# xx-peach/animatable_nerf

Measured on AMD Instinct MI355X. Metric: ray-samples/sec (512×512 rays × 64 samples) + PSNR, aninerf_s9p at 1/2/4/8 GPUs, higher is better.
Workload: dtype fp32; 1 GPU; aninerf_s9p full 512x512 render (config 2: fp32, novel-view eval, perturb=0); render_precision=fp32, rays_per_gpu=262142, samples_per_ray=64, chunk=2048, alpha_ind_rows=5863584, parallelism=replicas1 (one frame per GPU)

## Files before the change

animatable_nerf_amd/csrc/anr_mlp_body.h:

```cpp
#pragma once
#include <type_traits>

#include "anr_common.h"
#include "anr_kernels.h"
#include "anr_layers.h"

namespace anr {


template <int B, int E, typename F>
__device__ __forceinline__ void static_for(F&& f) {
  if constexpr (B < E) {
    f(std::integral_constant<int, B>{});
    static_for<B + 1, E>(f);
  }
}

typedef __attribute__((address_space(3))) void lds_void;
typedef __bf16 bf16x8 __attribute__((ext_vector_type(8)));
#ifndef ANR_FRAG_PF
#define ANR_FRAG_PF 3
#endif
#ifndef ANR_DMA_SPREAD
#define ANR_DMA_SPREAD 1
#endif
#ifndef ANR_X6_PF
#define ANR_X6_PF 2
#endif
#ifndef ANR_FAST_MATH
#define ANR_FAST_MATH 1
#endif

template <int V>
__host__ __device__ constexpr int prog_base() { return V >= 10 ? V - 10 : V; }
template <int V>
__host__ __device__ constexpr int prog_len() {
  constexpr int B = prog_base<V>();
  return B == 0 ? 30 : (B == 2 || B == 4) ? 28 : (B == 3 || B == 5) ? 9 : B == 7 ? 8 : B == 6 ? 5 : 18;
}
template <int V>
__host__ __device__ constexpr bool prog_seq() {
  return prog_base<V>() == 3 || prog_base<V>() == 5 || prog_base<V>() == 6 || prog_base<V>() == 7;
}
template <int V>
__host__ __device__ constexpr int prog_layer(int e) {
  if (V >= 10) return prog_layer<prog_base<V>()>(e);
  return V == 3 ? ANR_L_RESD0 + e
         : V == 5 ? ANR_L_SDF0 + e
         : V == 7 ? ANR_L_SREV0 + e
         : V == 6 ? ANR_L_COL0 + e
         : e < 9 ? e
         : V == 0 ? e - 9
         : (V == 2 || V == 4) ? (e < 26 ? e - 9 : (e == 26 ? ANR_L_HEAD : ANR_L_RGB))
         : V == 8 ? (e < 17 ? e : ANR_L_ALPHA)
                  : (e < 17 ? e : ANR_L_ALPHA);
}
__host__ __device__ constexpr bool prog_pose(int e) { return e < 9; }
template <bool B16, int V>
__host__ __device__ constexpr int prog_mode(int e) {
  return B16 ? ((V == 4 || V == 8 || V >= 10) ? 2 : e < 9 ? ANR_POSE_MODE : 1) : 0;
}
template <int V>
__host__ __device__ constexpr int prog_nobg(int e) { return (layer_desc_all(prog_layer<V>(e)).ob + 7) / 8; }
template <bool B16, int V>
__host__ __device__ constexpr int prog_slices(int e) {
  return prog_mode<B16, V>(e) == 2   ? ks32(prog_layer<V>(e)) * prog_nobg<V>(e)
         : prog_mode<B16, V>(e) == 1 ? ks32(prog_layer<V>(e)) + (b16_tail_ob(prog_layer<V>(e)) > 0 ? 1 : 0)
                                  : layer_ksteps(prog_layer<V>(e)) / ANR_KSLICE;
}
template <int V>
__host__ __device__ constexpr int x6_group_obs(int e, int gidx) {
  return layer_desc_all(prog_layer<V>(e)).ob - 8 * gidx < 8 ? layer_desc_all(prog_layer<V>(e)).ob - 8 * gidx : 8;
}
template <int V>
__host__ __device__ constexpr int x6_slice_of(int e, int G) {
  return (G / layer_desc_all(prog_layer<V>(e)).ob) * prog_nobg<V>(e) + (G % layer_desc_all(prog_layer<V>(e)).ob) / 8;
}
template <int V>
__host__ __device__ constexpr int x6_certified_at(int e, int F) {
  const int o = F % layer_desc_all(prog_layer<V>(e)).ob;
  const int gob = x6_group_obs<V>(e, o / 8);
  return x6_slice_of<V>(e, F) + (o % 8 > (gob - 1) / 2 ? 1 : 0);
}
template <int V>
__host__ __device__ constexpr int x6_issue_at(int e, int G) {
  int F = G - ANR_X6_PF > 0 ? G - ANR_X6_PF : 0;
  while (x6_certified_at<V>(e, F) < x6_slice_of<V>(e, G)) ++F;
  return F;
}
template <int V>
__host__ __device__ constexpr bool x6_schedule_ok(int e) {
  const int n = ks32(prog_layer<V>(e)) * layer_desc_all(prog_layer<V>(e)).ob;
  for (int G = 0; G < n; ++G) {
    const int F = x6_issue_at<V>(e, G);
    if (F > G || F < G - ANR_X6_PF) return false;
    if (x6_slice_of<V>(e, G) > x6_certified_at<V>(e, F)) return false;
    if (x6_slice_of<V>(e, G) > x6_slice_of<V>(e, F) + 1 || x6_slice_of<V>(e, G) < x6_slice_of<V>(e, F)) return false;
  }
  return true;
}
template <bool B16, int V>
__host__ __device__ constexpr int prog_slice_kb(int e, int q) {
  return prog_mode<B16, V>(e) == 2 ? x6_group_obs<V>(e, q % prog_nobg<V>(e)) * 3
         : prog_mode<B16, V>(e) == 1
             ? (q < ks32(prog_layer<V>(e)) ? b16_main_ob(prog_layer<V>(e)) * 2
                                          : b16_tail_ob(prog_layer<V>(e)) * ks32(prog_layer<V>(e)) * 2)
             : layer_chunks(prog_layer<V>(e)) * ANR_KSLICE;
}
template <bool B16, int V>
__host__ __device__ constexpr int prog_slice_off(int e, int q) {
  return prog_mode<B16, V>(e) == 2
             ? (prog_seq<V>() ? x6seq_layer_offset(prog_layer<V>(0), prog_layer<V>(e))
                              : x6_base() + x6_layer_offset(prog_layer<V>(e))) +
                   ((q / prog_nobg<V>(e)) * layer_desc_all(prog_layer<V>(e)).ob + 8 * (q % prog_nobg<V>(e))) * 3072
         : prog_mode<B16, V>(e) == 1
             ? (prog_seq<V>() ? seq_layer_offset(prog_layer<V>(0), prog_layer<V>(e))
                              : b16_base() + b16_layer_offset(prog_layer<V>(e))) +
                   q * b16_main_ob(prog_layer<V>(e)) * 2048
             : layer_offset(prog_layer<V>(e)) + q * layer_chunks(prog_layer<V>(e)) * ANR_KSLICE * 1024;
}
template <bool B16, int V>
__host__ __device__ constexpr int prog_slice_loads(int e, int q) { return (prog_slice_kb<B16, V>(e, q) + 7) / 8; }
template <bool B16, int V>
__host__ __device__ constexpr int prog_advance(int e, int q, int d) {
  for (int i = 0; i < d; ++i) {
    if (q + 1 < prog_slices<B16, V>(e)) {
      ++q;
    } else {
      q = 0;
      e = (e + 1) % prog_len<V>();
    }
  }
  return e * 1024 + q;
}
template <bool B16, int V>
__host__ __device__ constexpr int prog_later_loads(int e, int q) {
  int n = 0;
  for (int d = 1; d <= mlp_nbuf<B16>() - 3; ++d) {
    const int eq = prog_advance<B16, V>(e, q, d);
    n += prog_slice_loads<B16, V>(eq / 1024, eq % 1024);
  }
  return n;
}

template <int N>
__device__ __forceinline__ void wait_vmcnt() {
  static_assert(N >= 0 && N < 64, "vmcnt out of range");
  __builtin_amdgcn_s_waitcnt((N & 15) | (7 << 4) | (15 << 8) | ((N >> 4) << 14));
}

struct Pipe {
  unsigned char* lds;
  int smax;
  int nbuf;
  const unsigned char* wimg;
  int cur;
  int wave;
  int lane;
  int pose_woff;
  int pend;

  __device__ __forceinline__ void stage(int off, int kb, int loads, int buf, int first = 0) {
    const unsigned dst = (unsigned)(uintptr_t)(lds + buf * smax);
    const unsigned char* w = wimg;
    asm volatile("" : "+s"(w));
    for (int i = first; i < loads; ++i) {
      int piece = wave + 8 * i;
      piece = piece < kb ? piece : kb - 1;
      const unsigned m0 = dst + piece * 1024;
      const unsigned char* sbase = w + off + piece * 1024;
      asm volatile("s_mov_b32 m0, %2\n\ts_nop 0\n\tglobal_load_lds_dwordx4 %0, %1" ::"v"(lane * 16), "s"(sbase), "s"(m0)
                   : "memory");
    }
  }

  template <int N>
  __device__ __forceinline__ void wait_stream() {
    wait_vmcnt<N>();
  }

  template <bool B16, int V, int E, int Q>
  __device__ __forceinline__ void stage_slice(int buf) {
    constexpr int off = prog_slice_off<B16, V>(E, Q);
    stage(off + (prog_pose(E) ? pose_woff : 0), prog_slice_kb<B16, V>(E, Q), prog_slice_loads<B16, V>(E, Q), buf);
  }

  template <bool B16, int V>
  __device__ __forceinline__ void start() {
    static_for<0, mlp_nbuf<B16>() - 1>([&](auto d) {
      constexpr int eq = prog_advance<B16, V>(0, 0, decltype(d)::value);
      stage_slice<B16, V, eq / 1024, eq % 1024>(decltype(d)::value);
    });
    cur = 0;
    wait_stream<prog_later_loads<B16, V>(0, 0)>();
    __syncthreads();
  }

  template <bool B16, int V, int E, int Q>
  __device__ __forceinline__ const unsigned char* enter() {
    return lds + cur * smax;
  }
  template <bool B16, int V, int E, int Q, bool SPREAD = false>
  __device__ __forceinline__ void mid() {
    constexpr int NB = mlp_nbuf<B16>();
    constexpr int e1 = prog_advance<B16, V>(E, Q, 1);
    constexpr int eq = prog_advance<B16, V>(E, Q, NB - 1);
    wait_stream<prog_later_loads<B16, V>(e1 / 1024, e1 % 1024)>();
    __syncthreads();
    int slot = cur + NB - 1;
    slot = slot >= NB ? slot - NB : slot;
    if constexpr (SPREAD) pend = slot;
    else stage_slice<B16, V, eq / 1024, eq % 1024>(slot);
  }
  template <bool B16, int V, int E, int Q, int I0, int I1>
  __device__ __forceinline__ void piece() {
    constexpr int NB = mlp_nbuf<B16>();
    constexpr int eq = prog_advance<B16, V>(E, Q, NB - 1);
    constexpr int EE = eq / 1024, QQ = eq % 1024;
    constexpr int off = prog_slice_off<B16, V>(EE, QQ);
    constexpr int loads = prog_slice_loads<B16, V>(EE, QQ);
    constexpr int i1 = I1 < loads ? I1 : loads;
    if constexpr (I0 < i1) stage(off + (prog_pose(EE) ? pose_woff : 0), prog_slice_kb<B16, V>(EE, QQ), i1, pend, I0);
  }
  __device__ __forceinline__ void leave() { cur = cur + 1 >= nbuf ? 0 : cur + 1; }
};

__device__ __forceinline__ void split8(const float (&x)[8], bf16x8& hi, bf16x8& lo) {
#pragma unroll
  for (int j = 0; j < 8; ++j) {
    const __bf16 h = (__bf16)x[j];
    hi[j] = h;
    lo[j] = (__bf16)(x[j] - (float)h);
  }
}

__device__ __forceinline__ void split8x3(const float (&x)[8], bf16x8& hi, bf16x8& mid, bf16x8& lo) {
#pragma unroll
  for (int j = 0; j < 8; ++j) {
    const __bf16 h = (__bf16)x[j];
    const float r1 = x[j] - (float)h;
    const __bf16 m = (__bf16)r1;
    hi[j] = h;
    mid[j] = m;
    lo[j] = (__bf16)(r1 - (float)m);
  }
}

template <int V>
__host__ __device__ constexpr int prog_bias_off(int e) {
  int o = 0;
  for (int k = 0; k < e; ++k) o += layer_desc_all(prog_layer<V>(k)).ob * 16;
  return o;
}
static_assert(prog_bias_off<0>(prog_len<0>()) == ANR_BIAS_TABLE_FLOATS, "bias table size (anr_layers.h)");
static_assert(prog_bias_off<1>(prog_len<1>()) <= ANR_BIAS_TABLE_FLOATS, "bias table size (anr_layers.h)");
static_assert(prog_bias_off<2>(prog_len<2>()) <= ANR_BIAS_TABLE_FLOATS, "bias table size (anr_layers.h)");
static_assert(prog_bias_off<4>(prog_len<4>()) <= ANR_BIAS_TABLE_FLOATS, "bias table size (anr_layers.h)");
static_assert(prog_bias_off<8>(prog_len<8>()) <= ANR_BIAS_TABLE_FLOATS, "bias table size (anr_layers.h)");
static_assert(prog_bias_off<3>(prog_len<3>()) == seq_bias_off(ANR_L_RESD0, ANR_RESD_LAYERS), "resd bias section");
static_assert(prog_bias_off<5>(prog_len<5>()) == seq_bias_off(ANR_L_SDF0, ANR_SDF_LAYERS), "sdf bias section");
static_assert(prog_bias_off<5>(prog_len<5>()) <= ANR_BIAS_TABLE_FLOATS, "bias table size (anr_layers.h)");
static_assert(prog_bias_off<7>(prog_len<7>()) == seq_bias_off(ANR_L_SREV0, ANR_SREV_LAYERS), "sdf grad bias section");
static_assert(prog_bias_off<6>(prog_len<6>()) == seq_bias_off(ANR_L_COL0, ANR_COL_LAYERS), "colour bias section");
static_assert(prog_bias_off<7>(prog_len<7>()) + 256 <= ANR_BIAS_TABLE_FLOATS, "bias table + W8 row (anr_layers.h)");

template <int V>
__device__ __forceinline__ void fill_bias_table(const MlpArgs& a, float* __restrict__ sb, int tid) {
  static_for<0, prog_len<V>()>([&](auto ee) {
    constexpr int e = decltype(ee)::value;
    constexpr int L = prog_layer<V>(e);
    constexpr int n = layer_desc_all(L).ob * 16;
    constexpr int boff = bias_offset(L);
    constexpr int toff = prog_bias_off<V>(e);
    const float* src;
    constexpr int VB = prog_base<V>();
    if constexpr (VB == 3) {
      src = e == 0 ? a.fold : e == 5 ? a.fold + 256 : a.bias + toff;
    } else if constexpr (VB == 5 || VB == 7) {
      src = a.bias + toff;
    } else if constexpr (VB == 6) {
      src = e == 3 ? a.fold + 512 : a.bias + toff;
    } else if constexpr (e < 9) {
      src = L == 0 ? a.fold + 0 : L == 5 ? a.fold + 512 : a.bias + a.pose_boff + boff;
    } else if constexpr (V != 1 && V != 8 && e < 18) {
      src = L == 0 ? a.fold + 256 : L == 5 ? a.fold + 768 : a.bias + boff;
    } else {
      src = L == 18 ? a.fold + 1024 : L == ANR_L_HEAD ? a.fold + ANR_FOLD_HEAD : a.bias + boff;
    }
    for (int i = tid; i < n; i += 512) sb[toff + i] = src[i];
  });
}

#ifndef ANR_X3_STREAM
#define ANR_X3_STREAM 1
#endif
template <int L>
__host__ __device__ constexpr bool x3_stream_layer() {
  return ANR_X3_STREAM && b16_tail_ob(L) == 0;
}

template <int MOB, int PF>
__host__ __device__ constexpr int x3_issue_at(int G) {
  const int t = G / MOB;
  const int a = G - PF;
  if (t == 0) return a;
  const int m = (t - 1) * MOB + (MOB - 1) / 2;
  return a > m ? a : m;
}

struct LayerIO {
  float* spst = nullptr;
  const float* fst = nullptr;
  float fscale = 1.0f;
  const float* g0 = nullptr;
  const float* g1 = nullptr;
};

#ifndef ANR_SDF_NT
#define ANR_SDF_NT 1
#endif

__device__ __forceinline__ float softplus100(float x) {
  const float e = __builtin_amdgcn_exp2f(x * 144.269504f);
  const float h = __builtin_amdgcn_logf(1.0f + e) * 0.00693147181f;
  return x * 100.f > 20.f ? x : h;
}

__device__ __forceinline__ float softplus100_fac(float x, float& fac) {
  constexpr float C_HI = 144.26950073242188f, C_LO = 3.356474508109386e-06f;
  constexpr float LN2 = 0.6931471824645996f;
  const float xc = fminf(x, 0.4f);
  const float a = xc * C_HI;
  const float a_lo = __builtin_fmaf(xc, C_LO, __builtin_fmaf(xc, C_HI, -a));
  const float E = __builtin_amdgcn_exp2f(a);
  const float e = __builtin_fmaf(E, a_lo * LN2, E);
  const float u = 1.f + e;
  const float err = e - (u - 1.f);
  const float ru = __builtin_amdgcn_rcpf(u);
  fac = e * ru;
  return fmaxf(__builtin_fmaf(__builtin_amdgcn_logf(u), LN2, err * ru) * 0.01f, x);
}
template <int V>
__device__ __forceinline__ float sp_fwd(float x) {
  static_assert(V < 10, "the fp32-level programs use softplus100_fac");
  return softplus100(x);
}

template <bool B16, int V, int E, bool RELU_IN, int SP_IN, int FAC_IN, int NIN, int NOUT>
__device__ __forceinline__ void layer_x3(Pipe& p, const f32x4 (&in)[NIN], const float (&emb)[16], const float (&vemb)[8],
                                         f32x4 (&out)[NOUT], const float* __restrict__ sbias, int g, int lane,
                                         const LayerIO& io) {
  float* __restrict__ spst = io.spst;
  const float* __restrict__ fst = io.fst;
  const float fscale = io.fscale;
  constexpr int L = prog_layer<V>(E);
  constexpr LayerDesc D = layer_desc_all(L);
  constexpr int KS = ks32(L);
  constexpr int K0 = D.seg[0].ksteps / 8;
  constexpr int MOB = b16_main_ob(L);
  constexpr int PF = ANR_FRAG_PF;
  constexpr int NF = PF + 1;
  constexpr int MID = (MOB - 1) / 2;
  constexpr int BOFF = prog_bias_off<V>(E);
  static_assert(b16_tail_ob(L) == 0, "streamed x3 layers have no tail slice");
  f32x4 hv[2][2];
  auto load_h = [&](auto tc) {
    constexpr int t = decltype(tc)::value;
    if constexpr (FAC_IN != 0 && t < KS) {
#if ANR_SDF_NT
      hv[t & 1][0] = __builtin_nontemporal_load((const f32x4*)(fst + 32 * t + 4 * g));
      hv[t & 1][1] = __builtin_nontemporal_load((const f32x4*)(fst + 32 * t + 16 + 4 * g));
#else
      hv[t & 1][0] = *(const f32x4*)(fst + 32 * t + 4 * g);
      hv[t & 1][1] = *(const f32x4*)(fst + 32 * t + 16 + 4 * g);
#endif
    }
  };
// ... 224 lines not shown
          }
          load_h(std::integral_constant<int, tt + 1>{});
        }
        if constexpr (SP_IN != 0) {
          float* d = io.spst ? io.spst + 32 * ts + 4 * g : nullptr;
          const int c = 32 * ts + 4 * g;
#pragma unroll
          for (int q = 0; q < 2; ++q) {
            float f[4];
#pragma unroll
            for (int j = 0; j < 4; ++j) x[4 * q + j] = softplus100_fac(x[4 * q + j], f[j]);
            if (d) {
              if constexpr (SP_IN == 1) {
                __builtin_nontemporal_store(f32x4{f[0], f[1], f[2], f[3]}, (f32x4*)(d + 16 * q));
              } else {
#pragma unroll
                for (int j = 0; j < 4; ++j)
                  if (c + 16 * q + j < 217) d[16 * q + j] = f[j];
              }
            }
          }
        }
      }
      bf16x8 bh, bm, bl;
      split8x3(x, bh, bm, bl);
      static_for<0, OB>([&](auto ob) {
        constexpr int o = decltype(ob)::value;
        constexpr int F = tt * OB + o;
        constexpr int SQ = tt * NOBG + o / 8;
        if constexpr (o % 8 == 0) buf = p.template enter<B16, V, E, SQ>();
        if constexpr (tt == 0 && o == 0) init_bias();
        static_for<0, NS>([&](auto dd) {
          constexpr int G = F + decltype(dd)::value;
          if constexpr (G < KS * OB && x6_issue_at<V>(E, G) == F) {
            constexpr int og = G % OB;
            const unsigned char* src =
                x6_slice_of<V>(E, G) == SQ ? buf : p.lds + (p.cur + 1 >= p.nbuf ? 0 : p.cur + 1) * p.smax;
            fr[G % NS][0] = *(const bf16x8*)(src + (og % 8) * 3072 + lane * 16);
            fr[G % NS][1] = *(const bf16x8*)(src + (og % 8) * 3072 + 1024 + lane * 16);
            fr[G % NS][2] = *(const bf16x8*)(src + (og % 8) * 3072 + 2048 + lane * 16);
          }
        });
        __builtin_amdgcn_sched_barrier(0);
        const bf16x8 ah = fr[F % NS][0], am = fr[F % NS][1], al = fr[F % NS][2];
        out[o] = __builtin_amdgcn_mfma_f32_16x16x32_bf16(ah, bl, out[o], 0, 0, 0);
        out[o] = __builtin_amdgcn_mfma_f32_16x16x32_bf16(al, bh, out[o], 0, 0, 0);
        out[o] = __builtin_amdgcn_mfma_f32_16x16x32_bf16(am, bm, out[o], 0, 0, 0);
        out[o] = __builtin_amdgcn_mfma_f32_16x16x32_bf16(ah, bm, out[o], 0, 0, 0);
        out[o] = __builtin_amdgcn_mfma_f32_16x16x32_bf16(am, bh, out[o], 0, 0, 0);
        out[o] = __builtin_amdgcn_mfma_f32_16x16x32_bf16(ah, bh, out[o], 0, 0, 0);
        __builtin_amdgcn_sched_barrier(0);
        constexpr int GOB = x6_group_obs<V>(E, o / 8);
        if constexpr (o % 8 == (GOB - 1) / 2) p.template mid<B16, V, E, SQ>();
        if constexpr (o % 8 == GOB - 1) p.leave();
      });
    });
  } else if constexpr (prog_mode<B16, V>(E) != 0) {
    constexpr int KS = ks32(L);
    constexpr int K0 = D.seg[0].ksteps / 8;
    static_for<0, KS>([&](auto t) {
      constexpr int tt = decltype(t)::value;
      const unsigned char* buf = p.template enter<B16, V, E, tt>();
      if constexpr (tt == 0) init_bias();
      constexpr int seg = tt < K0 ? 0 : 1;
      constexpr int ts = tt < K0 ? tt : tt - K0;
      constexpr int kind = D.seg[seg].kind;
      float x[8];
      if constexpr (kind == SRC_EMB || kind == SRC_EMB6) {
#pragma unroll
        for (int j = 0; j < 8; ++j) x[j] = emb[8 * ts + j];
      } else if constexpr (kind == SRC_VEMB) {
#pragma unroll
        for (int j = 0; j < 8; ++j) x[j] = vemb[j];
      } else {
#pragma unroll
        for (int j = 0; j < 4; ++j) {
          x[j] = in[2 * ts][j];
          x[4 + j] = in[2 * ts + 1][j];
        }
      }
      {
        bf16x8 bh, bl;
        split8(x, bh, bl);
        constexpr int MOB = b16_main_ob(L);
        constexpr int PF = ANR_FRAG_PF;
        bf16x8 fh[PF + 1], fl[PF + 1];
        static_for<0, PF>([&](auto pp) {
          constexpr int o = decltype(pp)::value;
          if constexpr (o < MOB) {
            fh[o] = *(const bf16x8*)(buf + o * 2048 + lane * 16);
            fl[o] = *(const bf16x8*)(buf + o * 2048 + 1024 + lane * 16);
          }
        });
        static_for<0, MOB>([&](auto ob) {
          constexpr int o = decltype(ob)::value;
          constexpr int r = o % (PF + 1), rn = (o + PF) % (PF + 1);
          if constexpr (o + PF < MOB) {
            fh[rn] = *(const bf16x8*)(buf + (o + PF) * 2048 + lane * 16);
            fl[rn] = *(const bf16x8*)(buf + (o + PF) * 2048 + 1024 + lane * 16);
          }
          __builtin_amdgcn_sched_barrier(0);
          out[o] = __builtin_amdgcn_mfma_f32_16x16x32_bf16(fl[r], bh, out[o], 0, 0, 0);
          out[o] = __builtin_amdgcn_mfma_f32_16x16x32_bf16(fh[r], bl, out[o], 0, 0, 0);
          out[o] = __builtin_amdgcn_mfma_f32_16x16x32_bf16(fh[r], bh, out[o], 0, 0, 0);
          __builtin_amdgcn_sched_barrier(0);
          constexpr int MID = (MOB - 1) / 2;
          if constexpr (!ANR_DMA_SPREAD) {
            if constexpr (o == MID) p.template mid<B16, V, E, tt>();
          } else {
            constexpr int eqr = prog_advance<B16, V>(E, tt, mlp_nbuf<B16>() - 1);
            constexpr int NL = prog_slice_loads<B16, V>(eqr / 1024, eqr % 1024);
            constexpr int SPAN = MOB - 1 - MID;
            if constexpr (o == MID) p.template mid<B16, V, E, tt, true>();
            if constexpr (SPAN == 0) {
              if constexpr (o == MID) p.template piece<B16, V, E, tt, 0, NL>();
            } else if constexpr (o > MID) {
              constexpr int lo = ((o - MID - 1) * NL + SPAN - 1) / SPAN;
              constexpr int hi = o == MOB - 1 ? NL : ((o - MID) * NL + SPAN - 1) / SPAN;
              p.template piece<B16, V, E, tt, lo, hi>();
            }
          }
        });
        p.leave();
      }
    });
    if constexpr (b16_tail_ob(L) > 0) {
      constexpr int TOB = b16_tail_ob(L);
      const unsigned char* buf = p.template enter<B16, V, E, KS>();
      static_for<0, KS>([&](auto t) {
        constexpr int tt = decltype(t)::value;
        static_assert(D.nseg == 1 && D.seg[0].kind == SRC_ACT, "tail blocks only on activation-input layers");
        float x[8];
#pragma unroll
        for (int j = 0; j < 4; ++j) {
          x[j] = in[2 * tt][j];
          x[4 + j] = in[2 * tt + 1][j];
        }
        bf16x8 bh, bl;
        split8(x, bh, bl);
        static_for<0, TOB>([&](auto ob) {
          constexpr int o = decltype(ob)::value;
          const unsigned char* f = buf + (tt * TOB + o) * 2048 + lane * 16;
          const bf16x8 ah = *(const bf16x8*)f;
          const bf16x8 al = *(const bf16x8*)(f + 1024);
          out[16 + o] = __builtin_amdgcn_mfma_f32_16x16x32_bf16(al, bh, out[16 + o], 0, 0, 0);
          out[16 + o] = __builtin_amdgcn_mfma_f32_16x16x32_bf16(ah, bl, out[16 + o], 0, 0, 0);
          out[16 + o] = __builtin_amdgcn_mfma_f32_16x16x32_bf16(ah, bh, out[16 + o], 0, 0, 0);
        });
        if constexpr (tt == (KS - 1) / 2) p.template mid<B16, V, E, KS>();
      });
      p.leave();
    }
  } else {
    constexpr int C = layer_chunks(L);
    constexpr int K = layer_ksteps(L);
    constexpr int K0 = D.seg[0].ksteps;
    const unsigned char* buf = nullptr;
    static_for<0, K>([&](auto t) {
      constexpr int tt = decltype(t)::value;
      if constexpr (tt % ANR_KSLICE == 0) buf = p.template enter<B16, V, E, tt / ANR_KSLICE>();
      if constexpr (tt == 0) init_bias();
      f32x4 w[C];
      static_for<0, C>([&](auto c) {
        constexpr int cc = decltype(c)::value;
        w[cc] = *(const f32x4*)(buf + (((tt % ANR_KSLICE) * C + cc) * 64 + lane) * 16);
      });
      constexpr int seg = tt < K0 ? 0 : 1;
      constexpr int ts = tt < K0 ? tt : tt - K0;
      constexpr int kind = D.seg[seg].kind;
      float b;
      if constexpr (kind == SRC_EMB) b = emb[ts];
      else if constexpr (kind == SRC_VEMB) b = vemb[ts];
      else b = in[ts >> 2][ts & 3];
      static_for<0, D.ob>([&](auto ob) {
        constexpr int o = decltype(ob)::value;
        out[o] = __builtin_amdgcn_mfma_f32_16x16x4f32(w[o >> 2][o & 3], b, out[o], 0, 0, 0);
      });
      if constexpr (tt % ANR_KSLICE == ANR_KSLICE / 2 - 1) p.template mid<B16, V, E, tt / ANR_KSLICE>();
      if constexpr (tt % ANR_KSLICE == ANR_KSLICE - 1) p.leave();
    });
  }
  if constexpr (RELU) {
    static_for<0, D.ob>([&](auto ob) {
      constexpr int o = decltype(ob)::value;
#pragma unroll
      for (int r = 0; r < 4; ++r) out[o][r] = fmaxf(out[o][r], 0.0f);
    });
  }
}

__device__ __forceinline__ void sincos_fast(float x, float& s, float& c) {
  const float k = __builtin_rintf(x * 0.636619772367581343f);
  float r = __builtin_fmaf(-k, 1.57079601287841796875f, x);
  r = __builtin_fmaf(-k, 3.1391647326017846e-07f, r);
  r = __builtin_fmaf(-k, 5.3903025299577648e-15f, r);
  const float z = r * r;
  float ps = __builtin_fmaf(z, -1.9515295891e-4f, 8.3321608736e-3f);
  ps = __builtin_fmaf(ps, z, -1.6666654611e-1f);
  const float sn = __builtin_fmaf(ps * z, r, r);
  float pc = __builtin_fmaf(z, 2.443315711809948e-5f, -1.388731625493765e-3f);
  pc = __builtin_fmaf(pc, z, 4.166664568298827e-2f);
  pc = __builtin_fmaf(pc, z, -0.5f);
  const float cs = __builtin_fmaf(pc, z, 1.0f);
  const int q = (int)k;
  const float s0 = (q & 1) ? cs : sn, c0 = (q & 1) ? sn : cs;
  s = (q & 2) ? -s0 : s0;
  c = ((q + 1) & 2) ? -c0 : c0;
}

template <int NS>
__device__ __forceinline__ void embed_b(const float x[3], int h, int nfreq, float (&e)[8 * NS]) {
  asm volatile("" : "+v"(h));
  const float m = fmaxf(fabsf(x[0]), fmaxf(fabsf(x[1]), fabsf(x[2])));
  const bool slow = __builtin_amdgcn_ballot_w64(!(m * (float)(1 << (nfreq - 1)) <= 65536.0f)) != 0;
  const int hb = 4 * NS * h - 2;
#pragma unroll
  for (int s = 0; s < NS; ++s)
#pragma unroll
    for (int p = 0; p < 4; ++p) {
      const int P = hb + 4 * s + p;
      const int freq = (P * 11) >> 5;
      const int comp = P - 3 * freq;
      const float xc = comp == 0 ? x[0] : (comp == 1 ? x[1] : x[2]);
      const float arg = __builtin_ldexpf(xc, freq);
      float sv, cv;
      if (!slow) sincos_fast(arg, sv, cv);
      else sincosf(arg, &sv, &cv);
      const bool valid = (unsigned)P < (unsigned)(3 * nfreq);
      float v0 = valid ? sv : 0.0f, v1 = valid ? cv : 0.0f;
      if (s == 0 && p < 2) {
        const bool raw = h == 0;
        v0 = raw ? x[2 * p] : v0;
        v1 = raw ? (p == 0 ? x[1] : 0.0f) : v1;
      }
      e[8 * s + 2 * p] = v0;
      e[8 * s + 2 * p + 1] = v1;
    }
}

template <int NS>
__device__ __forceinline__ void embed(const float x[3], int g, int nfreq, float (&e)[NS]) {
#pragma unroll
  for (int s = 0; s < NS; ++s) {
    const int f = 4 * s + g;
    float v;
    if (f < 3) {
      v = x[f == 0 ? 0 : (f == 1 ? 1 : 2)];
    } else {
      const int q = f - 3;
      const int freq = q / 6;
      const int w = q - freq * 6;
      const int comp = w >= 3 ? w - 3 : w;
      const float xc = comp == 0 ? x[0] : (comp == 1 ? x[1] : x[2]);
      const float arg = xc * (float)(1 << (freq < 15 ? freq : 0));
      float sv, cv;
      sincosf(arg, &sv, &cv);
      v = freq >= nfreq ? 0.0f : (w >= 3 ? cv : sv);
    }
    e[s] = v;
  }
}

template <bool FAST = false>
__device__ __forceinline__ void lookup24(const float* __restrict__ vol32, const float p[3], const float* __restrict__ bounds,
                                         int X, int Y, int Z, int g, f32x4 (&out)[2]) {
#pragma clang fp contract(off)
  asm volatile("" : "+s"(X), "+s"(Y), "+s"(Z), "+s"(bounds));
  float lo[3], hi[3];
#pragma unroll
  for (int c = 0; c < 3; ++c) { lo[c] = bounds[c]; hi[c] = bounds[3 + c]; }
  TriCell t;
  if constexpr (FAST) {
    float gq[3];
#pragma unroll
    for (int c = 0; c < 3; ++c) gq[c] = (p[c] - lo[c]) * __builtin_amdgcn_rcpf(hi[c] - lo[c]) * 2.0f - 1.0f;
    const float ix = grid_src(gq[2], Z), iy = grid_src(gq[1], Y), iz = grid_src(gq[0], X);
    tri_cell_src(ix, iy, iz, X, Y, Z, t);
  } else {
    tri_cell(p, lo, hi, X, Y, Z, t);
  }
  f32x4 a0 = {0.f, 0.f, 0.f, 0.f}, a1 = {0.f, 0.f, 0.f, 0.f};
#pragma unroll
  for (int k = 0; k < 8; ++k) {
    if (t.base[k] >= 0) {
      const f32x4 v0 = *(const f32x4*)(vol32 + (size_t)t.base[k] * 32 + 4 * g);
      const f32x4 v1 = *(const f32x4*)(vol32 + (size_t)t.base[k] * 32 + 16 + 4 * g);
#pragma unroll
      for (int r = 0; r < 4; ++r) {
        a0[r] = a0[r] + v0[r] * t.w[k];
        a1[r] = a1[r] + v1[r] * t.w[k];
      }
    }
  }
  out[0] = a0;
  out[1] = a1;
}

template <bool FAST = false>
__device__ __forceinline__ void blend_softmax(const f32x4 (&fc)[2], const f32x4 (&init)[2], int g, f32x4 (&bw)[2]) {
  float lg[2][4];
  float m = -INFINITY;
#pragma unroll
  for (int b = 0; b < 2; ++b)
#pragma unroll
    for (int r = 0; r < 4; ++r) {
      const bool valid = b == 0 || g < 2;
      const float v = (FAST ? __logf(init[b][r] + 1e-9f) : logf(init[b][r] + 1e-9f)) + fc[b][r];
      lg[b][r] = valid ? v : -INFINITY;
      m = fmaxf(m, lg[b][r]);
    }
  m = fmaxf(m, __shfl_xor(m, 16));
  m = fmaxf(m, __shfl_xor(m, 32));
  float s = 0.f;
#pragma unroll
  for (int b = 0; b < 2; ++b)
#pragma unroll
    for (int r = 0; r < 4; ++r) {
      lg[b][r] = FAST ? __expf(lg[b][r] - m) : expf(lg[b][r] - m);
      s += lg[b][r];
    }
  s += __shfl_xor(s, 16);
  s += __shfl_xor(s, 32);
#pragma unroll
  for (int b = 0; b < 2; ++b)
#pragma unroll
    for (int r = 0; r < 4; ++r) bw[b][r] = FAST ? lg[b][r] * __builtin_amdgcn_rcpf(s) : lg[b][r] / s;
}

__device__ __forceinline__ void lbs_inverse(const f32x4 (&bw)[2], const float* __restrict__ sA, int g, const float x[3],
                                            float xt[3]) {
  float Ab[16];
#pragma unroll
  for (int m = 0; m < 16; ++m) Ab[m] = 0.f;
#pragma unroll
  for (int b = 0; b < 2; ++b)
#pragma unroll
    for (int r = 0; r < 4; ++r) {
      const int j = b * 16 + 4 * g + r;
      if (j < 24) {
        const float wj = bw[b][r];
#pragma unroll
        for (int m = 0; m < 16; ++m) Ab[m] += wj * sA[j * 16 + m];
      }
    }
#pragma unroll
  for (int m = 0; m < 16; ++m) {
    Ab[m] += __shfl_xor(Ab[m], 16);
    Ab[m] += __shfl_xor(Ab[m], 32);
  }
  const float a = Ab[0], b = Ab[1], c = Ab[2], d = Ab[4], e = Ab[5], f = Ab[6], gg = Ab[8], h = Ab[9], i = Ab[10];
  const float c00 = e * i - f * h, c01 = c * h - b * i, c02 = b * f - c * e;
  const float c10 = f * gg - d * i, c11 = a * i - c * gg, c12 = c * d - a * f;
  const float c20 = d * h - e * gg, c21 = b * gg - a * h, c22 = a * e - b * d;
  const float det = a * c00 + b * c10 + c * c20;
  const float rd = 1.0f / det;
  const float y0 = x[0] - Ab[3], y1 = x[1] - Ab[7], y2 = x[2] - Ab[11];
  xt[0] = (c00 * rd) * y0 + (c01 * rd) * y1 + (c02 * rd) * y2;
  xt[1] = (c10 * rd) * y0 + (c11 * rd) * y1 + (c12 * rd) * y2;
  xt[2] = (c20 * rd) * y0 + (c21 * rd) * y1 + (c22 * rd) * y2;
}

__device__ __forceinline__ void store_rows(float* __restrict__ rows, int idx, const f32x4 (&bw)[2], int g, bool valid) {
  if (!valid) return;
  *(f32x4*)(rows + (size_t)idx * 24 + 4 * g) = bw[0];
  if (g < 2) *(f32x4*)(rows + (size_t)idx * 24 + 16 + 4 * g) = bw[1];
}

template <bool B16, int V, int E0>
__device__ __forceinline__ void bw_mlp(Pipe& p, const float (&emb)[16], const float (&vemb)[8], const float* __restrict__ sb,
                                       f32x4 (&A)[17], f32x4 (&B)[17], f32x4 (&fc)[2], int g, int lane) {
  f32x4 dummy[1];
  layer<B16, V, E0 + 0, true>(p, dummy, emb, vemb, A, sb, g, lane);
  layer<B16, V, E0 + 1, true, true>(p, A, emb, vemb, B, sb, g, lane);
  layer<B16, V, E0 + 2, true, true>(p, B, emb, vemb, A, sb, g, lane);
  layer<B16, V, E0 + 3, true, true>(p, A, emb, vemb, B, sb, g, lane);
  layer<B16, V, E0 + 4, true, true>(p, B, emb, vemb, A, sb, g, lane);
  layer<B16, V, E0 + 5, true, true>(p, A, emb, vemb, B, sb, g, lane);
  layer<B16, V, E0 + 6, true, true>(p, B, emb, vemb, A, sb, g, lane);
  layer<B16, V, E0 + 7, true, true>(p, A, emb, vemb, B, sb, g, lane);
  layer<B16, V, E0 + 8, false, true>(p, B, emb, vemb, fc, sb, g, lane);
}

template <bool B16, int V = 2>
__device__ __forceinline__ void mlp_body(const MlpArgs& a) {
  static_assert(V == 2 || V == 4, "render programs");
  constexpr bool FAST = B16 && ANR_FAST_MATH && V == 2;
  extern __shared__ __attribute__((aligned(16))) unsigned char smem[];
  const int tid = threadIdx.x;
  const int lane = tid & 63;
  const int wave = __builtin_amdgcn_readfirstlane(tid >> 6);
  const int g = lane >> 4;
  const int pl = lane & 15;
  float* sb = (float*)smem;
  float* sA = (float*)(smem + mlp_sa_off());
  for (int i = tid; i < 384; i += 512) sA[i] = a.A[i];
  fill_bias_table<V>(a, sb, tid);

  float* sT = sA + 384;
  if (tid < 6) sT[tid] = a.tbounds[tid];
  const int n = *a.n_kept;
  const int ntiles = (n + 127) / 128;
  if ((int)blockIdx.x >= ntiles) return;

  Pipe p{smem + mlp_ring_off(), mlp_slice_max<B16>(), mlp_nbuf<B16>(), a.wimg, 0, wave, lane, a.pose_woff};
  p.template start<B16, V>();

  for (int tile = blockIdx.x; tile < ntiles; tile += gridDim.x) {
    const int idx = tile * 128 + wave * 16 + pl;
    const bool valid = idx < n;
    const int pid = a.list[valid ? idx : n - 1];
    float dist, pose[3], dir[3];
    if (a.dists) {
      world_to_pose_pt(a.wpts, pid, a.n_pts, a.chunk_pts, a.R, a.Th, pose);
      dist = a.dists[pid];
#pragma unroll
      for (int c = 0; c < 3; ++c) dir[c] = a.vdir[3 * (size_t)pid + c];
    } else {
      const int ray = pid >> 6, s = pid & 63;
      float z, pts[3];
      sample_point(a.ray_o, a.ray_d, a.near_, a.far_, a.t_rand, ray, s, 64, z, dist, pts);
      world_to_pose(pts, a.R, a.Th, pose);
#pragma unroll
      for (int c = 0; c < 3; ++c) dir[c] = a.ray_d[3 * ray + c];
    }

    float emb[16], vemb[8];
    f32x4 A[17], B[17], fc[2], init[2], bw[2];

    if constexpr (B16) embed_b<2>(pose, g, 10, emb);
    else embed<16>(pose, g, 10, emb);
    lookup24<FAST>(a.pbw32, pose, a.pbounds, a.pX, a.pY, a.pZ, g, init);
#pragma unroll
    for (int s8 = 0; s8 < 8; ++s8) vemb[s8] = 0.f;
    bw_mlp<B16, V, 0>(p, emb, vemb, sb, A, B, fc, g, lane);
    blend_softmax<FAST>(fc, init, g, bw);
    store_rows(a.pbw_rows, idx, bw, g, valid);
    float xt[3];
    lbs_inverse(bw, sA, g, pose, xt);

    if constexpr (B16) embed_b<2>(xt, g, 10, emb);
    else embed<16>(xt, g, 10, emb);
    lookup24<FAST>(a.tbw32, xt, a.tbounds, a.tX, a.tY, a.tZ, g, init);
    bw_mlp<B16, V, 9>(p, emb, vemb, sb, A, B, fc, g, lane);
    blend_softmax<FAST>(fc, init, g, bw);
    store_rows(a.tbw_rows, idx, bw, g, valid);

    f32x4 dummy[1];
    layer<B16, V, 18, true>(p, dummy, emb, vemb, A, sb, g, lane);
    layer<B16, V, 19, true, true>(p, A, emb, vemb, B, sb, g, lane);
    layer<B16, V, 20, true, true>(p, B, emb, vemb, A, sb, g, lane);
    layer<B16, V, 21, true, true>(p, A, emb, vemb, B, sb, g, lane);
    layer<B16, V, 22, true, true>(p, B, emb, vemb, A, sb, g, lane);
    layer<B16, V, 23, true, true>(p, A, emb, vemb, B, sb, g, lane);
    layer<B16, V, 24, true, true>(p, B, emb, vemb, A, sb, g, lane);
    layer<B16, V, 25, true, true>(p, A, emb, vemb, B, sb, g, lane);
    float sigma_raw;
    if constexpr (B16) embed_b<1>(dir, g, 4, vemb);
    else embed<8>(dir, g, 4, vemb);
    layer<B16, V, 26, false, true>(p, B, emb, vemb, A, sb, g, lane);
    sigma_raw = __shfl(A[8][0], pl);
    if constexpr (!(prog_mode<B16, V>(27) == 1 && x3_stream_layer<ANR_L_RGB>())) {
      static_for<0, 8>([&](auto ob) {
        constexpr int o = decltype(ob)::value;
#pragma unroll
        for (int r = 0; r < 4; ++r) A[o][r] = fmaxf(A[o][r], 0.0f);
      });
    }
    layer<B16, V, 27, false, true>(p, A, emb, vemb, B, sb, g, lane);

    bool inside = true;
#pragma unroll
    for (int c = 0; c < 3; ++c) inside = inside && (xt[c] > sT[c]) && (xt[c] < sT[3 + c]);
    const float sig = inside ? sigma_raw : 0.0f;
    if (valid && g == 0) {
      float4 r;
      r.x = 1.0f / (1.0f + expf(-B[0][0]));
      r.y = 1.0f / (1.0f + expf(-B[0][1]));
      r.z = 1.0f / (1.0f + expf(-B[0][2]));
      r.w = 1.0f - expf(-fmaxf(sig, 0.0f) * dist);
      a.raw[pid] = r;
      a.sigma[idx] = sig;
    }
  }
  asm volatile("s_waitcnt vmcnt(0)" ::: "memory");
}

template <bool B16, int V = 1>
__device__ __forceinline__ void alpha_body(const MlpArgs& a) {
  static_assert(V == 1 || V == 8, "density programs");
  constexpr bool FAST = B16 && ANR_FAST_MATH && V == 1;
  extern __shared__ __attribute__((aligned(16))) unsigned char smem[];
  const int tid = threadIdx.x;
  const int lane = tid & 63;
  const int wave = __builtin_amdgcn_readfirstlane(tid >> 6);
  const int g = lane >> 4;
  const int pl = lane & 15;
  float* sb = (float*)smem;
  float* sA = (float*)(smem + mlp_sa_off());
  for (int i = tid; i < 384; i += 512) sA[i] = a.A[i];
  fill_bias_table<V>(a, sb, tid);

  const int n = *a.n_kept;
  const int ntiles = (n + 127) / 128;
  if ((int)blockIdx.x >= ntiles) return;

  Pipe p{smem + mlp_ring_off(), mlp_slice_max<B16>(), mlp_nbuf<B16>(), a.wimg, 0, wave, lane, a.pose_woff};
  p.template start<B16, V>();

  for (int tile = blockIdx.x; tile < ntiles; tile += gridDim.x) {
    const int idx = tile * 128 + wave * 16 + pl;
    const bool valid = idx < n;
    const int pid = a.list[valid ? idx : n - 1];
    float pose[3];
    world_to_pose_pt(a.wpts, pid, a.n_pts, a.chunk_pts, a.R, a.Th, pose);

    float emb[16], vemb[8];
    f32x4 A[17], B[17], fc[2], init[2], bw[2];
    if constexpr (B16) embed_b<2>(pose, g, 10, emb);
    else embed<16>(pose, g, 10, emb);
    lookup24<FAST>(a.pbw32, pose, a.pbounds, a.pX, a.pY, a.pZ, g, init);
#pragma unroll
    for (int s8 = 0; s8 < 8; ++s8) vemb[s8] = 0.f;
    bw_mlp<B16, V, 0>(p, emb, vemb, sb, A, B, fc, g, lane);
    blend_softmax<FAST>(fc, init, g, bw);
    float xt[3];
    lbs_inverse(bw, sA, g, pose, xt);

    if constexpr (B16) embed_b<2>(xt, g, 10, emb);
    else embed<16>(xt, g, 10, emb);
    f32x4 dummy[1];
    layer<B16, V, 9, true>(p, dummy, emb, vemb, A, sb, g, lane);
    layer<B16, V, 10, true, true>(p, A, emb, vemb, B, sb, g, lane);
    layer<B16, V, 11, true, true>(p, B, emb, vemb, A, sb, g, lane);
    layer<B16, V, 12, true, true>(p, A, emb, vemb, B, sb, g, lane);
    layer<B16, V, 13, true, true>(p, B, emb, vemb, A, sb, g, lane);
    layer<B16, V, 14, true, true>(p, A, emb, vemb, B, sb, g, lane);
    layer<B16, V, 15, true, true>(p, B, emb, vemb, A, sb, g, lane);
    layer<B16, V, 16, true, true>(p, A, emb, vemb, B, sb, g, lane);
    layer<B16, V, 17, false, true>(p, B, emb, vemb, A, sb, g, lane);
    if (valid && g == 0) a.alpha_out[pid] = A[0][0];
  }
  asm volatile("s_waitcnt vmcnt(0)" ::: "memory");
}

template <bool X6>
__device__ __forceinline__ void resd_body(const MlpArgs& a) {
  constexpr int V = 3 + (X6 ? 10 : 0);
  extern __shared__ __attribute__((aligned(16))) unsigned char smem[];
  const int tid = threadIdx.x;
  const int lane = tid & 63;
  const int wave = __builtin_amdgcn_readfirstlane(tid >> 6);
  const int g = lane >> 4;
  const int pl = lane & 15;
  float* sb = (float*)smem;
  fill_bias_table<V>(a, sb, tid);
  const int n = a.n_rows;
  const int ntiles = (n + 127) / 128;
  if ((int)blockIdx.x >= ntiles) return;

  Pipe p{smem + mlp_ring_off(), mlp_slice_max<true>(), mlp_nbuf<true>(), a.wimg, 0, wave, lane, 0};
  p.template start<true, V>();

  for (int tile = blockIdx.x; tile < ntiles; tile += gridDim.x) {
    const int idx = tile * 128 + wave * 16 + pl;
    const bool valid = idx < n;
    const float* pt = a.ptb + (size_t)(valid ? idx : n - 1) * a.ptb_ld;
    const float x[3] = {pt[0], pt[1], pt[2]};
    float emb[16], vemb[8];
    f32x4 A[17], B[17], fc[2];
    embed_b<2>(x, g, 10, emb);
#pragma unroll
    for (int s8 = 0; s8 < 8; ++s8) vemb[s8] = 0.f;
    bw_mlp<true, V, 0>(p, emb, vemb, sb, A, B, fc, g, lane);
    if (valid && g == 0) {
      float* y = a.yr + (size_t)idx * 4;
      y[0] = fc[0][0];
      y[1] = fc[0][1];
      y[2] = fc[0][2];
    }
  }
  asm volatile("s_waitcnt vmcnt(0)" ::: "memory");
}

template <int NOB, int V>
__device__ __forceinline__ void softplus_regs(f32x4 (&v)[17]) {
  static_for<0, NOB>([&](auto ob) {
    constexpr int o = decltype(ob)::value;
#pragma unroll
    for (int r = 0; r < 4; ++r) v[o][r] = sp_fwd<V>(v[o][r]);
  });
}

template <bool X6>
__device__ __forceinline__ void sdfnet_body(const MlpArgs& a) {
  constexpr int V = 5 + (X6 ? 10 : 0);
  extern __shared__ __attribute__((aligned(16))) unsigned char smem[];
  const int tid = threadIdx.x;
  const int lane = tid & 63;
  const int wave = __builtin_amdgcn_readfirstlane(tid >> 6);
  const int g = lane >> 4;
  const int pl = lane & 15;
  float* sb = (float*)smem;
  fill_bias_table<V>(a, sb, tid);
  const int n = a.n_rows;
  const int ntiles = (n + 127) / 128;
  if ((int)blockIdx.x >= ntiles) return;

  Pipe p{smem + mlp_ring_off(), mlp_slice_max<true>(), mlp_nbuf<true>(), a.wimg, 0, wave, lane, 0};
  p.template start<true, V>();

  for (int tile = blockIdx.x; tile < ntiles; tile += gridDim.x) {
    const int idx = tile * 128 + wave * 16 + pl;
    const bool valid = idx < n;
    const size_t row = (size_t)(valid ? idx : n - 1);
    const float* pt = a.ptb + row * a.ptb_ld;
    const float x[3] = {pt[0], pt[1], pt[2]};
    float emb[16], vemb[8];
    f32x4 A[17], B[17];
    embed_b<2>(x, g, 6, emb);
#pragma unroll
    for (int s8 = 0; s8 < 8; ++s8) vemb[s8] = 0.f;
    auto store_h = [&](const f32x4(&v)[17], float* __restrict__ dst) {
      if (!valid) return;
      float* d = dst + row * 256 + 4 * g;
      static_for<0, 16>([&](auto ob) {
        constexpr int o = decltype(ob)::value;
        *(f32x4*)(d + 16 * o) = v[o];
      });
    };
    auto st = [&](int i) { return LayerIO{valid ? (i == 3 ? a.x4 : a.sdf_h[i]) + row * 256 : nullptr}; };
    f32x4 dummy[1];
    layer<true, V, 0, false>(p, dummy, emb, vemb, A, sb, g, lane);
    layer<true, V, 1, false, false, 1>(p, A, emb, vemb, B, sb, g, lane, st(0));
    layer<true, V, 2, false, false, 1>(p, B, emb, vemb, A, sb, g, lane, st(1));
    layer<true, V, 3, false, false, 1>(p, A, emb, vemb, B, sb, g, lane, st(2));
    layer<true, V, 4, false, false, 2>(p, B, emb, vemb, A, sb, g, lane, st(3));
    layer<true, V, 5, false, false, 1>(p, A, emb, vemb, B, sb, g, lane, st(4));
    layer<true, V, 6, false, false, 1>(p, B, emb, vemb, A, sb, g, lane, st(5));
    layer<true, V, 7, false, false, 1>(p, A, emb, vemb, B, sb, g, lane, st(6));
    if constexpr (X6) {
      float* d = a.sdf_h[7] + row * 256 + 4 * g;
      static_for<0, 16>([&](auto ob) {
        constexpr int o = decltype(ob)::value;
        float f[4];
#pragma unroll
        for (int r = 0; r < 4; ++r) B[o][r] = softplus100_fac(B[o][r], f[r]);
        if (valid) *(f32x4*)(d + 16 * o) = f32x4{f[0], f[1], f[2], f[3]};
      });
    } else {
      softplus_regs<16, V>(B);
      store_h(B, a.sdf_h[7]);
    }
    layer<true, V, 8, false>(p, B, emb, vemb, A, sb, g, lane);
    if (valid) {
      float* d = a.y8 + row * 264;
      static_for<0, 17>([&](auto ob) {
        constexpr int o = decltype(ob)::value;
#pragma unroll
        for (int r = 0; r < 4; ++r) {
          const int m = 16 * o + 4 * g + r;
// ... 133 lines not shown
```

Before: 120.8 million ray-samples/s.

## Software-pipeline fp32 MLP weight fragment reads across k-steps and layers

In the fp32 MFMA path, weight fragments are now held in the pipeline struct and the next k-step's (or next layer's) fragments are read from LDS chunk by chunk, interleaved with the current MFMAs behind scheduling barriers. The first layer's fragments are primed before the tile loop, and DMA staging of upcoming slices is spread across the late k-steps instead of issued at the mid point. The aim is to hide LDS read latency and smooth global-to-LDS traffic. In exchange it adds register pressure and relies on a compile-time check that the prefetch never reads an uncertified ring slot.

```diff
diff --git a/animatable_nerf_amd/csrc/anr_mlp_body.h b/animatable_nerf_amd/csrc/anr_mlp_body.h
--- a/animatable_nerf_amd/csrc/anr_mlp_body.h
+++ b/animatable_nerf_amd/csrc/anr_mlp_body.h
@@ -30,6 +30,13 @@
 #ifndef ANR_FAST_MATH
 #define ANR_FAST_MATH 1
 #endif
+#define ANR_F32_WMAX 5
+#ifndef ANR_F32_XLAYER
+#define ANR_F32_XLAYER 1
+#endif
+#ifndef ANR_F32_DMA_SPREAD
+#define ANR_F32_DMA_SPREAD 1
+#endif
 
 template <int V>
 __host__ __device__ constexpr int prog_base() { return V >= 10 ? V - 10 : V; }
@@ -143,6 +150,22 @@
   return n;
 }
 
+template <int V>
+__host__ __device__ constexpr bool f32_stream_ok() {
+  constexpr int F32_MID = ANR_KSLICE / 2 - 1;
+  int n = 0;
+  for (int e = 0; e < prog_len<V>(); ++e) {
+    if (layer_ksteps(prog_layer<V>(e)) % ANR_KSLICE != 0) return false;
+    if (layer_chunks(prog_layer<V>(e)) > ANR_F32_WMAX) return false;
+    n += layer_ksteps(prog_layer<V>(e));
+  }
+  for (int i = 0; i < n; ++i) {
+    const int s = i / ANR_KSLICE, s1 = (i + 1) / ANR_KSLICE;
+    if (s1 != s && !(s1 == s + 1 && i % ANR_KSLICE > F32_MID)) return false;
+    if (i + 1 >= (s1 + 1) * ANR_KSLICE + F32_MID) return false;
+  }
+  return mlp_nbuf<false>() >= 3;
+}
 template <int N>
 __device__ __forceinline__ void wait_vmcnt() {
   static_assert(N >= 0 && N < 64, "vmcnt out of range");
@@ -159,6 +182,7 @@
   int lane;
   int pose_woff;
   int pend;
+  f32x4 w[ANR_F32_WMAX];
 
   __device__ __forceinline__ void stage(int off, int kb, int loads, int buf, int first = 0) {
     const unsigned dst = (unsigned)(uintptr_t)(lds + buf * smax);
@@ -223,6 +247,19 @@
     if constexpr (I0 < i1) stage(off + (prog_pose(EE) ? pose_woff : 0), prog_slice_kb<B16, V>(EE, QQ), i1, pend, I0);
   }
   __device__ __forceinline__ void leave() { cur = cur + 1 >= nbuf ? 0 : cur + 1; }
+  template <int C, int KS, int C0, int C1, bool NEXT>
+  __device__ __forceinline__ void read_w() {
+    const unsigned char* src = lds + (NEXT ? (cur + 1 >= nbuf ? 0 : cur + 1) : cur) * smax;
+    static_for<C0, C1>([&](auto c) {
+      constexpr int cc = decltype(c)::value;
+      w[cc] = *(const f32x4*)(src + ((KS * C + cc) * 64 + lane) * 16);
+    });
+  }
+  template <int V>
+  __device__ __forceinline__ void prime_f32() {
+    constexpr int C = layer_chunks(prog_layer<V>(0));
+    read_w<C, 0, 0, C, false>();
+  }
 };
 
 __device__ __forceinline__ void split8(const float (&x)[8], bf16x8& hi, bf16x8& lo) {
@@ -753,19 +790,21 @@
       p.leave();
     }
   } else {
+    static_assert(f32_stream_ok<V>(), "fp32 fragment stream reads an uncertified slice");
     constexpr int C = layer_chunks(L);
     constexpr int K = layer_ksteps(L);
     constexpr int K0 = D.seg[0].ksteps;
-    const unsigned char* buf = nullptr;
+    constexpr int CN = layer_chunks(prog_layer<V>((E + 1) % prog_len<V>()));
     static_for<0, K>([&](auto t) {
       constexpr int tt = decltype(t)::value;
-      if constexpr (tt % ANR_KSLICE == 0) buf = p.template enter<B16, V, E, tt / ANR_KSLICE>();
-      if constexpr (tt == 0) init_bias();
-      f32x4 w[C];
-      static_for<0, C>([&](auto c) {
-        constexpr int cc = decltype(c)::value;
-        w[cc] = *(const f32x4*)(buf + (((tt % ANR_KSLICE) * C + cc) * 64 + lane) * 16);
-      });
+      constexpr int ks = tt % ANR_KSLICE;
+      constexpr int Q = tt / ANR_KSLICE;
+      constexpr int MIDK = ANR_KSLICE / 2 - 1;
+      if constexpr (ks == 0) p.template enter<B16, V, E, Q>();
+      if constexpr (tt == 0) {
+        init_bias();
+        if constexpr (!ANR_F32_XLAYER) p.template read_w<C, 0, 0, C, false>();
+      }
       constexpr int seg = tt < K0 ? 0 : 1;
       constexpr int ts = tt < K0 ? tt : tt - K0;
       constexpr int kind = D.seg[seg].kind;
@@ -773,12 +812,29 @@
       if constexpr (kind == SRC_EMB) b = emb[ts];
       else if constexpr (kind == SRC_VEMB) b = vemb[ts];
       else b = in[ts >> 2][ts & 3];
-      static_for<0, D.ob>([&](auto ob) {
-        constexpr int o = decltype(ob)::value;
-        out[o] = __builtin_amdgcn_mfma_f32_16x16x4f32(w[o >> 2][o & 3], b, out[o], 0, 0, 0);
+      constexpr bool LAST = tt == K - 1;
+      constexpr int NC = !LAST ? C : ANR_F32_XLAYER ? CN : 0;
+      constexpr int NCC = LAST ? CN : C;
+      constexpr bool NEXT = ks == ANR_KSLICE - 1;
+      constexpr int NKS = NEXT ? 0 : ks + 1;
+      static_for<0, C>([&](auto c) {
+        constexpr int cc = decltype(c)::value;
+        static_for<4 * cc, (4 * cc + 4 < D.ob ? 4 * cc + 4 : D.ob)>([&](auto ob) {
+          constexpr int o = decltype(ob)::value;
+          out[o] = __builtin_amdgcn_mfma_f32_16x16x4f32(p.w[cc][o & 3], b, out[o], 0, 0, 0);
+        });
+        __builtin_amdgcn_sched_barrier(0);
+        if constexpr (cc < NC) p.template read_w<NCC, NKS, cc, cc + 1, NEXT>();
+        if constexpr (ANR_F32_DMA_SPREAD && cc == 0 && ks > MIDK) {
+          constexpr int eqr = prog_advance<B16, V>(E, Q, mlp_nbuf<B16>() - 1);
+          constexpr int NL = prog_slice_loads<B16, V>(eqr / 1024, eqr % 1024);
+          p.template piece<B16, V, E, Q, ks - MIDK - 1, (NEXT ? NL : ks - MIDK)>();
+        }
+        __builtin_amdgcn_sched_barrier(0);
       });
-      if constexpr (tt % ANR_KSLICE == ANR_KSLICE / 2 - 1) p.template mid<B16, V, E, tt / ANR_KSLICE>();
-      if constexpr (tt % ANR_KSLICE == ANR_KSLICE - 1) p.leave();
+      if constexpr (NC > C) p.template read_w<NCC, NKS, C, NC, NEXT>();
+      if constexpr (ks == MIDK) p.template mid<B16, V, E, Q, ANR_F32_DMA_SPREAD != 0>();
+      if constexpr (NEXT) p.leave();
     });
   }
   if constexpr (RELU) {
@@ -1005,6 +1061,7 @@
 
   Pipe p{smem + mlp_ring_off(), mlp_slice_max<B16>(), mlp_nbuf<B16>(), a.wimg, 0, wave, lane, a.pose_woff};
   p.template start<B16, V>();
+  if constexpr (!B16 && ANR_F32_XLAYER) p.template prime_f32<V>();
 
   for (int tile = blockIdx.x; tile < ntiles; tile += gridDim.x) {
     const int idx = tile * 128 + wave * 16 + pl;
@@ -1107,6 +1164,7 @@
 
   Pipe p{smem + mlp_ring_off(), mlp_slice_max<B16>(), mlp_nbuf<B16>(), a.wimg, 0, wave, lane, a.pose_woff};
   p.template start<B16, V>();
+  if constexpr (!B16 && ANR_F32_XLAYER) p.template prime_f32<V>();
 
   for (int tile = blockIdx.x; tile < ntiles; tile += gridDim.x) {
     const int idx = tile * 128 + wave * 16 + pl;
```

Result: faster. 124.7 million ray-samples/s (median of 6 runs) (+3.2%).
